# AlexandreRouma/SDRPlusPlus

Hardware: NVIDIA H100
Metric: complex IQ MSamples/s through FFT + 8-VFO WFM chain (higher is better)
Workload: dtype f32

## Files before the change

### sdrplusplus_b200/csrc/api.cpp

```cpp
#include "../../include/b200dsp.h"
#include "engine.h"
#include <chrono>
#include <map>
#include <cmath>
#include <cstdio>
#include <cstring>
#include <cstdlib>
#include <algorithm>

using namespace b200;

static int g_device = -1;

static int ensure_device() {
    int n = 0;
    cudaError_t e = cudaGetDeviceCount(&n);
    if (e != cudaSuccess || n <= 0) {
        set_error("no usable CUDA device (%s): libb200dsp has no CPU fallback", e == cudaSuccess ? "0 devices" : cudaGetErrorString(e));
        cudaGetLastError();
        return B200_ENODEV;
    }
    if (g_device < 0) { g_device = 0; }
    B200_CK(cudaSetDevice(g_device));
    return 0;
// ... 417 lines not shown
extern "C" int b200_fe_vfo_max_out(b200_fe* fe, int id, int count) {
    VfoSlot* v = get_vfo(fe, id);
    if (!v) { return B200_EINVAL; }
    return v->chain.max_out(count);
}
extern "C" int b200_fe_fft_max_lines(b200_fe* fe, int count) {
    if (!fe || !fe->fft_on) { return 0; }
    return (int)(count / ((long long)fe->fft.nz + fe->skip)) + 2;
}
extern "C" long long b200_fe_launch_count(b200_fe* fe) { return fe ? fe->sch.launches : 0; }
extern int g_xd_tma_launches;
extern "C" long long b200_fe_stat(b200_fe* fe, const char* key) {
    if (!fe || !key) { return -1; }
    if (!strcmp(key, "launches")) { return fe->sch.launches; }
    if (!strcmp(key, "s1_tma_launches")) { return g_xd_tma_launches; }
    if (!strcmp(key, "chunks")) { return (long long)fe->nsub; }
    if (!strcmp(key, "host_ns_plan")) { return fe->host_ns[0]; }
    if (!strcmp(key, "host_ns_fft")) { return fe->host_ns[1]; }
    if (!strcmp(key, "host_ns_run")) { return fe->host_ns[2]; }
    if (!strcmp(key, "host_ns_join")) { return fe->host_ns[3]; }
    if (!strcmp(key, "graph_hits")) { return fe->sch.graph_hits; }
    if (!strcmp(key, "graph_misses")) { return fe->sch.graph_misses; }
    if (!strcmp(key, "graphs")) { return (long long)fe->sch.graphs.size(); }
    if (!strcmp(key, "host_ns_stage1")) { return fe->sch.host_ns[0]; }
    if (!strcmp(key, "host_ns_tail")) { return fe->sch.host_ns[1]; }
    return -1;
}
extern "C" int b200_fe_set_option(b200_fe* fe, const char* key, int value) {
    if (!fe || !key) { set_error("null argument"); return B200_EINVAL; }
    if (!strcmp(key, "s1")) { fe->sch.s1_variant = value; return 0; }
    if (!strcmp(key, "overlap")) {
        if (b200_fe_vfo_count(fe) > 0) { set_error("'overlap' must be chosen before VFOs are added"); return B200_ESTATE; }
        if (cudaDeviceSynchronize() != cudaSuccess) { return cuda_fail(cudaGetLastError(), "sync"); }
        fe->sch.tail_stream = value ? fe->tail_stream : nullptr;
        return 0;
    }
    if (!strcmp(key, "pair")) { fe->sch.pair_conjugates = value != 0; return 0; }
    if (!strcmp(key, "fft_async")) { fe->fft_async = value != 0; return 0; }
    if (!strcmp(key, "s1_mt")) { kernels_set_xd_tile(value); return 0; }
    if (!strcmp(key, "s1_cps")) { kernels_set_xd_cps(value); return 0; }
    if (!strcmp(key, "s1_stages")) { kernels_set_xd_tma_stages(value); return 0; }
    if (!strcmp(key, "s1_diag")) { kernels_set_xd_tma_diag(value); return 0; }
    if (!strcmp(key, "s1_ctas")) { kernels_set_xd_tma_ctas(value); return 0; }
    if (!strcmp(key, "tails") || !strncmp(key, "ft_", 3)) {
        if (b200_fe_vfo_count(fe) > 0) { set_error("'%s' must be chosen before VFOs are added", key); return B200_ESTATE; }
        if (!strcmp(key, "tails")) { kernels_set_tail_variant(value >= 1 ? 1 : 0); fe->sch.fuse.on = value >= 2; return 0; }
        if (!strcmp(key, "ft_ob")) { fe->sch.fuse.ob_force = value; return 0; }
        if (!strcmp(key, "ft_obmax")) { fe->sch.fuse.ob_max = value; return 0; }
        if (!strcmp(key, "ft_smem_kb")) { fe->sch.fuse.smem_limit = value * 1024; return 0; }
        if (!strcmp(key, "ft_threads")) { fe->sch.fuse.threads = value; return 0; }
        if (!strcmp(key, "ft_direct")) { fe->sch.fuse.direct = value != 0; return 0; }
        if (!strcmp(key, "ft_prereg")) { fe->sch.fuse.pre_reg = value; return 0; }
        if (!strcmp(key, "ft_regall")) { fe->sch.fuse.reg_all = value != 0; return 0; }
// ... 1127 lines not shown
```

### sdrplusplus_b200/csrc/engine.cpp

```cpp
#include "engine.h"
#include <chrono>
#include "../../include/b200dsp.h"
#include <cmath>
#include <cstdarg>
#include <cstdio>
#include <cstring>
#include <algorithm>
#include <map>
#include <functional>
#include <cstdlib>

namespace b200 {

static thread_local char g_err[512] = "";
void set_error(const char* fmt, ...) {
    va_list ap;
    va_start(ap, fmt);
    vsnprintf(g_err, sizeof(g_err), fmt, ap);
    va_end(ap);
}
const char* last_error() { return g_err; }
int cuda_fail(cudaError_t e, const char* what) {
    set_error("CUDA error %d (%s) in %s", (int)e, cudaGetErrorString(e), what);
    if (e == cudaErrorNoDevice || e == cudaErrorInsufficientDriver) { return B200_ENODEV; }
// ... 288 lines not shown
    memset(init_state, 0, sizeof(init_state));
    init_state[7] = 1.0f;
    int rc = state.alloc(sizeof(init_state));
    if (rc) { return rc; }
    B200_CK(cudaMemcpy(state.p, init_state, sizeof(init_state), cudaMemcpyHostToDevice));
    return 0;
}
int FmIfStage::configure(int nbins) {
    if (!fmif_supported(nbins)) { set_error("FM IF noise reduction: %d bins (supported: 2 ... %d)", nbins, 64); return B200_EINVAL; }
    bins = nbins;
    hist = bins - 1;
    const std::vector<float> w = fmif_window(bins), t = dft_twiddles(bins);
    int rc;
    if ((rc = win.alloc(w.size() * sizeof(float), false)) || (rc = tw.alloc(t.size() * sizeof(float), false))) { return rc; }
    B200_CK(cudaMemcpy(win.p, w.data(), w.size() * sizeof(float), cudaMemcpyHostToDevice));
    B200_CK(cudaMemcpy(tw.p, t.data(), t.size() * sizeof(float), cudaMemcpyHostToDevice));
    return 0;
}

int Chain::finalize(int max_in, bool dbl_first, const FuseCfg* fuse) {
    if (st.empty()) { set_error("empty chain"); return B200_EINVAL; }
    int cap = max_in;
    if (dbl_first && st.size() >= 2 && st[0]->kind == K_XD) { st[1]->dbl = true; }
    for (auto& s : st) {
        if (s->kind != K_XD) {
            int rc = s->alloc_in(cap);
            if (rc) { return rc; }
        }
        else { s->cap_in = cap; }
        cap = s->max_out(cap);
    }
    {
        int c2 = max_in;
        for (auto& s : st) {
            if (s->kind == K_STEREO) {
                StereoStage* q = (StereoStage*)s.get();
                int rc2;
                if ((rc2 = q->p.alloc(((size_t)c2 + 8) * sizeof(float2), false)) || (rc2 = q->vco.alloc(((size_t)c2 + 8) * sizeof(float2), false))) { return rc2; }
            }
            c2 = s->max_out(c2);
        }
    }
    out_es = st.back()->out_es;
    out_cap = cap;
    int rc = out.alloc(((size_t)cap + 8) * out_es * sizeof(float));
    if (rc) { return rc; }
// ... 663 lines not shown
    }
    for (Chain* c : chains) {
        for (auto& sp : c->st) { sp->par = parity; }
    }
    if (tail_stream && chunk_idx >= 2) {
        B200_CK(cudaStreamWaitEvent(stream, ev_tail[parity], 0));
    }
    trace_mark("stage1 start", stream);
    for (Chain* c : chains) {
        depth = std::max(depth, c->st.size());
        for (size_t i = 0; i < c->st.size(); i++) {
            Stage* s = c->st[i].get();
            s->out_ptr = (i + 1 < c->st.size()) ? c->st[i + 1]->in_data() : (c->out_override ? c->out_override : c->out.as<float>());
            if (s->kind == K_XD) {
                XdStage* x = (XdStage*)s;
                if (x->taps_dirty) {
                    int rc = x->upload_taps(stream);
                    if (rc) { return rc; }
                }
            }
        }
    }
    std::map<int, std::vector<XdStage*>> groups;
    for (Chain* c : chains) {
        if (c->raw_input()) {
            XdStage* x = (XdStage*)c->st[0].get();
            groups[x->D].push_back(x);
        }
    }
    for (auto& kv : groups) {
        std::vector<XdStage*>& g = kv.second;
        for (size_t b = 0; b < g.size(); b += B200_BATCH) {
            XdParams p;
            memset(&p, 0, sizeof(p));
            p.in = raw;
            p.hist = raw_hist.as<float2>();
            p.hist_len = RAW_HIST;
            p.count = count;
            p.D = kv.first;
            p.in_scale = in_scale;
            p.QP = 1;
            p.njobs = (int)std::min<size_t>(B200_BATCH, g.size() - b);
            for (int v = 0; v < p.njobs; v++) {
                XdStage* x = g[b + v];
                p.job[v].out = (float2*)x->out_ptr;
                p.job[v].gpad = x->gpad.as<float2>();
                p.job[v].phase0 = x->chunk_phase0;
                p.job[v].w = x->w;
                p.job[v].offset = x->chunk_offset;
                p.job[v].n_out = x->n_out;
                p.job[v].T = x->T;
                p.job[v].h = x->hdev.as<float>();
                p.job[v].w_prev = x->chunk_w_prev;
                p.job[v].retuned = x->chunk_retuned ? 1 : 0;
// ... 42 lines not shown
                            const unsigned long long r = g[b + v]->w * (unsigned long long)P;
                            const double d0 = (double)(long long)r;
                            const double d1 = (double)(long long)(r - 0x8000000000000000ULL);
                            int sv = 0;
                            if (std::fabs(d0) <= tol) { sv = 1; } else if (std::fabs(d1) <= tol) { sv = -1; }
                            if (sv == 0 || (sg != 0 && sv != sg)) { ok = false; }
                            sg = sv;
                        }
                        if (!ok) { continue; }
                        for (int PS : { 8, 10 }) {
                            if (PS % P == 0) {
                                p.pfb_ps = PS;
                                p.pfb_sigma = (sg < 0 && ((PS / P) & 1)) ? -1 : 1;
                                break;
                            }
                        }
                    }
                }
            }
            int variant = s1_variant;
            for (int v = 0; v < p.njobs; v++) {
                if (g[b + v]->gpad_len < (p.D - 1) + (p.QP + 8) * p.D) { variant = 0; }
            }
            int nl = 0;
            cudaEvent_t t1 = timer_begin(0, stream);
            cudaError_t e = launch_xlate_decim(p, fmt, variant, stream, &nl);
            if (e != cudaSuccess) { return cuda_fail(e, "launch_xlate_decim"); }
            if (t1) { B200_CK(cudaEventRecord(t1, stream)); }
            trace_mark("stage1 done", stream);
            e = launch_xd_edge(p, fmt, stream, &nl);
            if (e != cudaSuccess) { return cuda_fail(e, "launch_xd_edge"); }
            launches += nl;
        }
    }
    if (carry_raw && count > 0) {
        CarryParams rc1;
        rc1.njobs = 1;
        CarryJob& j = rc1.job[0];
        j.dst = raw_hist.as<float>(); j.a = raw_hist.as<float>(); j.b = raw;
        j.h = RAW_HIST; j.la = RAW_HIST; j.lb = count; j.esize = 2; j.bfmt = fmt; j.scale = in_scale;
        cudaError_t e = launch_carry(rc1, stream);
        if (e != cudaSuccess) { return cuda_fail(e, "launch_carry"); }
        launches++;
    }
    if (tail_stream) {
        B200_CK(cudaEventRecord(ev_stage1[parity], stream));
        B200_CK(cudaStreamWaitEvent(ts, ev_stage1[parity], 0));
    }
    trace_mark("tails start", ts);
// ... 26 lines not shown
            int rc = dfr_flush();
            if (rc) { return rc; }
        }
        if (dfr.njobs == 0) {
            dfr_D = f->decim; dfr_T = f->ntaps; dfr_taps = &f->htaps;
            memcpy(dfr.taps, f->htaps.data(), (size_t)f->ntaps * sizeof(float));
        }
        FirJob& j = dfr.job[dfr.njobs++];
        j.in = (const float2*)f->base(); j.out = (float2*)f->out_ptr; j.taps = f->taps.as<float>();
        j.ntaps = f->ntaps; j.decim = f->decim; j.offset = f->chunk_offset; j.n_out = f->n_out;
        dfr.max_out = std::max(dfr.max_out, f->n_out);
        return 0;
    };
    auto dfr_ok = [&](const Stage* s) {
        if (fuse.pre_reg <= 0 || s->kind != K_FIRC || s->in_es != 2) { return false; }
        const FirCStage* f = (const FirCStage*)s;
        return f->decim > 1 && f->ntaps <= DFR_MAXT && dfir_reg_supported(f->decim, f->ntaps);
    };
    {
        int max_beg = 1;
        for (Chain* c : chains) { if (c->fp.active) { max_beg = std::max(max_beg, c->fp.beg); } }
        for (int lvl = 1; lvl < max_beg; lvl++) {
            for (Chain* c : chains) {
                if (!c->fp.active || lvl >= c->fp.beg) { continue; }
                FirCStage* f = (FirCStage*)c->st[lvl].get();
                if (f->n_out <= 0) { continue; }
                int rc = dfr_push(f);
                if (rc) { return rc; }
            }
            int rc = dfr_flush();
            if (rc) { return rc; }
        }
    }
    {
        std::vector<Chain*> fc;
        for (Chain* c : chains) {
            if (c->fp.active && c->st[c->fp.beg]->n_in > 0) { fc.push_back(c); }
        }
        if (!fc.empty()) {
            const int threads = (fuse.threads == 512 || fuse.threads == 256) ? fuse.threads : 128;
            size_t smem = 0;
            int ob_cap = 1 << 30;
            for (Chain* c : fc) { smem = std::max(smem, c->fp.smem); ob_cap = std::min(ob_cap, c->fp.ob_max); }
            static std::map<std::pair<int, size_t>, int> occ_cache;
            int cps;
            {
                auto key = std::make_pair(threads, smem);
// ... 110 lines not shown
            else {
                cudaError_t e = launch_squelch(sqp, ts, &nl);
                if (e != cudaSuccess) { return cuda_fail(e, "launch_squelch"); }
            }
            launches += nl;
            sqp.njobs = 0; sqp.max_n = 0;
            return 0;
        };
        auto st_flush = [&]() -> int {
            if (stp.njobs == 0) { return 0; }
            int nl = 0;
            if (g_rec) { g_rec->add(LaunchRec::T_STEREO, nullptr, &stp, sizeof(stp)); }
            else {
                cudaError_t e = launch_stereo(stp, ts, &nl);
                if (e != cudaSuccess) { return cuda_fail(e, "launch_stereo"); }
            }
            launches += nl;
            stp.njobs = 0; stp.max_n = 0;
            return 0;
        };
        for (Chain* c : chains) {
            if (lvl >= c->st.size()) { continue; }
            if (c->fp.active && lvl >= 1 && (int)lvl < c->fp.end) { continue; }
            Stage* s = c->st[lvl].get();
            int rc = 0;
            switch (s->kind) {
            case K_XD: break;
            case K_FIRC: {
                FirCStage* f = (FirCStage*)s;
                if (f->n_out <= 0) { break; }
                if (dfr_ok(f)) { rc = dfr_push(f); break; }
                if (fuse.pre_reg > 0 && f->decim == 1 && f->in_es == 2 && f->ntaps <= 2000 && f->chunk_offset == 0) {
                    FirJob& jr = fpr.job[fpr.njobs++];
                    jr.in = (const float2*)f->base(); jr.out = (float2*)f->out_ptr; jr.taps = f->taps.as<float>();
                    jr.ntaps = f->ntaps; jr.decim = 1; jr.offset = 0; jr.n_out = f->n_out;
                    fpr.max_out = std::max(fpr.max_out, f->n_out);
                    if (fpr.njobs == B200_BATCH) { rc = flush_batch(fpr, launch_fir_reg, ts, launches); fpr.max_out = 0; }
                    break;
                }
                FirJob& j = fp.job[fp.njobs++];
                j.in = (const float2*)f->base(); j.out = (float2*)f->out_ptr; j.taps = f->taps.as<float>();
                j.ntaps = f->ntaps; j.decim = f->decim; j.offset = f->chunk_offset; j.n_out = f->n_out;
                fp.max_out = std::max(fp.max_out, f->n_out);
                if (fp.njobs == B200_BATCH) { rc = flush_batch(fp, launch_fir_c, ts, launches); fp.max_out = 0; }
                break;
            }
// ... 126 lines not shown
        if ((rc = flush_batch(fp, launch_fir_c, ts, launches))) { return rc; }
        if ((rc = flush_batch(pp, launch_poly, ts, launches))) { return rc; }
        if ((rc = flush_batch(qp, launch_quad, ts, launches))) { return rc; }
        if ((rc = flush_batch(rp, launch_fir_r, ts, launches))) { return rc; }
        if ((rc = flush_batch(sp, launch_seq, ts, launches))) { return rc; }
        if ((rc = flush_batch(mp, launch_m2s, ts, launches))) { return rc; }
        if ((rc = flush_batch(cp2, launch_scale, ts, launches))) { return rc; }
        if ((rc = flush_batch(fmp, launch_fmif, ts, launches))) { return rc; }
        if ((rc = flush_batch(xlp, launch_rxl, ts, launches))) { return rc; }
        if ((rc = st_flush())) { return rc; }
        if ((rc = sq_flush())) { return rc; }
    }
    CarryParams cp;
    zero_params(cp, use_rec);
    auto push = [&](const CarryJob& j) -> int {
        cp.job[cp.njobs++] = j;
        if (cp.njobs == CARRY_BATCH) { return flush_batch(cp, launch_carry, ts, launches); }
        return 0;
    };
    for (Chain* c : chains) {
        for (auto& sp : c->st) {
            Stage* s = sp.get();
            if (s->kind == K_XD || s->hist <= 0 || s->fmid) { continue; }
            if (s->n_in <= 0 && !s->dbl) { continue; }
            CarryJob j;
            memset(&j, 0, sizeof(j));
            j.dst = s->other_base(); j.a = s->base(); j.b = s->in_data();
            j.h = s->hist; j.la = s->hist; j.lb = s->n_in; j.esize = s->in_es; j.bfmt = -1; j.scale = 0.0f;
            int rc = push(j);
            if (rc) { return rc; }
        }
    }
    int rcf = flush_batch(cp, launch_carry, ts, launches);
    if (rcf) { return rcf; }
    return 0;
    };
    if (nsplit == 1) {
        rec.cur_branch = 0;
        int rcs = tail_section(all_chains);
        if (rcs) { return rcs; }
    }
    else {
        const size_t half = (all_chains.size() + 1) / 2;
        std::vector<Chain*> ga(all_chains.begin(), all_chains.begin() + half), gb(all_chains.begin() + half, all_chains.end());
        rec.cur_branch = 0;
        int rcs = tail_section(ga);
// ... 20 lines not shown
```

### sdrplusplus_b200/csrc/engine.h

```cpp
#pragma once
#include <cuda_runtime.h>
#include <cstdint>
#include <memory>
#include <mutex>
#include <string>
#include <vector>
#include <unordered_map>
#include "kernels.cuh"
#include "design.h"

namespace b200 {

void trace_mark(const char* label, cudaStream_t s);
void trace_dump(const char* title);
bool trace_on();

void set_error(const char* fmt, ...);
const char* last_error();
int cuda_fail(cudaError_t e, const char* what);
#define B200_CK(call)                                                     \
    do {                                                                  \
        cudaError_t _e = (call);                                          \
        if (_e != cudaSuccess) { return b200::cuda_fail(_e, #call); }     \
    } while (0)
// ... 164 lines not shown
    DevBuf win, tw;
    FmIfStage() { kind = K_FMIF; in_es = 2; out_es = 2; }
    int configure(int nbins);
    int plan(int n) override { n_in = n; n_out = n; return n; }
    int max_out(int n) const override { return n; }
};

struct ScaleStage : Stage {
    float gain = 1.0f;
    ScaleStage(int es, float g) { kind = K_SCALE; in_es = es; out_es = es; gain = g; }
    int plan(int n) override { n_in = n; n_out = n; return n; }
    int max_out(int n) const override { return n; }
};

struct Chain {
    std::vector<std::unique_ptr<Stage>> st;
    DevBuf out;
    int out_es = 2;
    int out_cap = 0;
    int n_out = 0;
    float* out_override = nullptr;
    bool raw_input() const { return !st.empty() && st[0]->kind == K_XD; }
    int chan_fir = -1;
    FusedPlan fp;
    FuseCfg fcfg;
    int plan_fused();
    int finalize(int max_in, bool dbl_first = false, const FuseCfg* fuse = nullptr);
    int plan(int n);
    int max_out(int n) const;
    int peek(int n) const;
    void reset_state();
    int add_rxvfo(double inSR, double outSR, double bw, double offset);
    int add_xlator(double offsetHz, double samplerate);
    int add_power_decim(int ratio);
    int add_resampler(double inSR, double outSR);
    int add_fir_c(const std::vector<float>& taps, int decim);
    int add_fir_r(const std::vector<float>& taps, bool stereo);
    int add_quad(double deviationHz, double samplerate);
    int add_wfm(double deviationHz, double samplerate, bool lowPass, bool stereo = false);
    int add_nfm(double samplerate, double bandwidth, bool lowPass);
    int add_am(int agcMode, double bandwidth, double attack, double decay, double dcRate, double samplerate);
    int add_ssb(int mode, double bandwidth, double samplerate, double attack, double decay);
    int add_deemph(double tau, double samplerate);
    int add_af_chain(double afSamplerate, double audioSamplerate, bool highPass, double deemphTau);
    int add_wfm_rds(double deviationHz, double samplerate);
    int add_noise_blanker(double rate, double level);
// ... 16 lines not shown
    int replay(cudaStream_t s, long long* nlaunch) const;
};

struct Scheduler {
    cudaStream_t stream = nullptr;
    cudaStream_t tail_stream = nullptr;
    cudaEvent_t ev_stage1[2] = { nullptr, nullptr }, ev_tail[2] = { nullptr, nullptr };
    unsigned long long chunk_idx = 0;
    cudaStream_t out_stream() const { return tail_stream ? tail_stream : stream; }
    int enable_overlap(cudaStream_t tail);
    long long launches = 0;
    int graph_tails = -1;
    int graph_max_count = 1 << 30;
    int tail_split = 1;
    cudaStream_t tail_stream2 = nullptr;
    struct GraphEntry { cudaGraphExec_t exec = nullptr; long long launches = 0; std::vector<unsigned char> key; };
    std::unordered_map<unsigned long long, GraphEntry> graphs;
    LaunchRec rec;
    long long graph_hits = 0, graph_misses = 0;
    void drop_graphs();
    int launch_recorded(cudaStream_t ts, bool may_graph);
    long long host_ns[4] = { 0, 0, 0, 0 };
    int s1_variant = 8;
    FuseCfg fuse;
    int sm_count = 132;
    float in_scale = 1.0f / 32768.0f;
    bool pair_conjugates = true;
    bool time_s1 = false;
    static const size_t TIMER_MAX = 512;
    struct Timer { std::vector<cudaEvent_t> ev; size_t used = 0; };
    Timer timers[3];
    cudaEvent_t timer_begin(int group, cudaStream_t s);
    int group_stats(int group, double* ms_total, int* launches);
    int s1_stats(double* ms_total, int* launches) { return group_stats(0, ms_total, launches); }
    ~Scheduler();
    DevBuf raw_hist;
    static const int RAW_HIST = 1024;
    static const int STAGE_SPARE = 72;
    int init_raw();
    int run(std::vector<Chain*>& chains, const void* raw, int fmt, int count, bool carry_raw);
    int apply_deferred(std::vector<Chain*>& chains);
    int reset_raw();
};

}
```

### sdrplusplus_b200/csrc/kernels.cu

```cuda
#include "kernels.cuh"
#include <unordered_map>
#include <mutex>
#include <math.h>
#include <string.h>
#include <algorithm>

template <int FMT>
__device__ __forceinline__ float2 load_iq(const void* __restrict__ p, long long i, float sc) {
    if (FMT == FMT_CF32) {
        return __ldg(reinterpret_cast<const float2*>(p) + i);
    }
    else if (FMT == FMT_CS16) {
        short2 v = __ldg(reinterpret_cast<const short2*>(p) + i);
        return make_float2((float)v.x * sc, (float)v.y * sc);
    }
    else {
        char2 v = __ldg(reinterpret_cast<const char2*>(p) + i);
        return make_float2((float)v.x * sc, (float)v.y * sc);
    }
}

template <int FMT>
__device__ __forceinline__ float2 load_x(const XdParams& p, long long i) {
    if (i >= 0) {
// ... 758 lines not shown

typedef CUresult (*PFN_tmap_encode)(CUtensorMap*, CUtensorMapDataType, cuuint32_t, void*, const cuuint64_t*, const cuuint64_t*,
                                    const cuuint32_t*, const cuuint32_t*, CUtensorMapInterleave, CUtensorMapSwizzle,
                                    CUtensorMapL2promotion, CUtensorMapFloatOOBfill);
static PFN_tmap_encode tmap_encode_fn() {
    static PFN_tmap_encode fn = nullptr;
    static bool tried = false;
    if (!tried) {
        tried = true;
        void* f = nullptr;
        cudaDriverEntryPointQueryResult q;
        if (cudaGetDriverEntryPoint("cuTensorMapEncodeTiled", &f, cudaEnableDefault, &q) == cudaSuccess && q == cudaDriverEntryPointSuccess) {
            fn = (PFN_tmap_encode)f;
        }
        else { cudaGetLastError(); }
    }
    return fn;
}
int g_xd_tma_launches = 0;
int g_xd_tma_stages = 2;
void kernels_set_xd_tma_stages(int n) { g_xd_tma_stages = (n == 3) ? 3 : 2; }
static int g_xd_tma_diag = 0;
void kernels_set_xd_tma_diag(int v) { g_xd_tma_diag = v & 3; }
template <int LOGD, int QC, int PS, int MT, int NST>
static cudaError_t launch_xd_tma_n(const XdParams& p, const XtGeom& g, const CUtensorMap& tm, cudaStream_t s) {
    using Lay = XtLay<LOGD, QC, MT>;
    const size_t smem = (size_t)NST * Lay::STAGE + ((size_t)B200_BATCH * (PS + 16) + (size_t)Lay::NW * B200_BATCH * 4) * sizeof(float2) +
                        2 * NST * sizeof(unsigned long long) + 1024;
    if ((int)smem > kernels_max_smem_optin()) { return cudaErrorInvalidValue; }
    static bool attr_set = false;
    if (!attr_set) {
        cudaError_t e = set_smem(k_xd_tma<LOGD, QC, PS, MT, NST>, smem);
        if (e != cudaSuccess) { return e; }
        attr_set = true;
    }
    int grid = num_sms();
    if (g_xd_tma_ctas > 0 && g_xd_tma_ctas < grid) { grid = g_xd_tma_ctas; }
    if (grid > g.ntiles) { grid = g.ntiles; }
    k_xd_tma<LOGD, QC, PS, MT, NST><<<grid, (Lay::NW + 1) * 32, smem, s>>>(p, g, tm);
    g_xd_tma_launches++;
    return cudaGetLastError();
}
template <int LOGD, int QC, int PS, int MT>
static cudaError_t launch_xd_tma_t(const XdParams& p, const XtGeom& g, const CUtensorMap& tm, cudaStream_t s) {
    return g_xd_tma_stages == 3 ? launch_xd_tma_n<LOGD, QC, PS, MT, 3>(p, g, tm, s) : launch_xd_tma_n<LOGD, QC, PS, MT, 2>(p, g, tm, s);
}
static bool try_xd_tma(const XdParams& p, cudaStream_t s, cudaError_t* err) {
    const int D = p.D, PS = p.pfb_ps;
    if ((PS != 8 && PS != 10) || (D != 32 && D != 64) || !p.taps_host) { return false; }
    if (((uintptr_t)p.in & 15) != 0) { return false; }
    PFN_tmap_encode enc = tmap_encode_fn();
    if (!enc) { return false; }
    const int T = p.job[0].T;
    const int a0 = p.job[0].offset - (T - 1);
    const int org = ((a0 % D) + D) % D;
    for (int v = 0; v < p.njobs; v++) {
        const int a = p.job[v].offset - (p.job[v].T - 1);
        if (p.job[v].T != T || a != a0 || p.job[v].n_out != p.job[0].n_out || p.job[v].n_out <= 0) { return false; }
    }
    const int QC = (T + (org & 1) + D - 1) / D;
    int sh = org & 1;
    for (int al = 16; al >= 2; al >>= 1) {
        const int c = org & (al - 1);
        if ((T + c + D - 1) / D == QC) { sh = c; break; }
    }
    if (QC * D > XT_MAXTAPS) { return false; }
    XtGeom g;
// ... 414 lines not shown
```

### sdrplusplus_b200/csrc/kernels.cuh

```cuda
#pragma once
#include <cuda_runtime.h>
#include <stdint.h>

#define B200_BATCH 16

enum { FMT_CF32 = 0, FMT_CS16 = 1, FMT_CS8 = 2 };

struct XdJob {
    float2* out;
    const float2* gpad;
    unsigned long long phase0;
    unsigned long long w;
    int offset;
    int n_out;
    int T;
    const float* h;
    unsigned long long w_prev;
    int retuned;
};
struct XdParams {
    const void* in;
    const float2* hist;
    int hist_len;
    int count;
    int D;
    int QP;
    int njobs;
    int nslots;
    signed char slot_a[B200_BATCH], slot_b[B200_BATCH];
    int pfb_ps, pfb_sigma;
    float in_scale;
    const float* taps_host;
    XdJob job[B200_BATCH];
};

struct FirJob {
    const float2* in;
    float2* out;
    const float* taps;
    int ntaps, decim, offset, n_out;
};
struct FirParams { int njobs; int max_out; FirJob job[B200_BATCH]; };

#define DFR_THREADS 128
#define DFR_MAXT 72

struct DfrParams {
    int njobs;
    int max_out;
    float taps[DFR_MAXT];
    FirJob job[B200_BATCH];
};

bool dfir_reg_supported(int D, int T);
cudaError_t launch_dfir_reg(const DfrParams& p, int D, int T, cudaStream_t s);

// ... 277 lines not shown
```

### sdrplusplus_b200/csrc/xd_tma.cuh

```cuda
#pragma once
#include <cuda.h>

#define XT_STAGES NST
#define XT_MAXTAPS 512

struct XtGeom {
    float g[XT_MAXTAPS];
    long long jmin;
    int ntiles;
    int org;
    int s;
    int cj;
    int rows_tma;
    int diag;
};

__device__ __forceinline__ void xt_mbar_init(unsigned bar, int count) {
    asm volatile("mbarrier.init.shared::cta.b64 [%0], %1;\n" ::"r"(bar), "r"(count) : "memory");
}
__device__ __forceinline__ void xt_mbar_wait(unsigned bar, unsigned parity) {
    asm volatile("{\n.reg .pred p;\nXT_WAIT_%=:\nmbarrier.try_wait.parity.shared::cta.b64 p, [%0], %1;\n@!p bra XT_WAIT_%=;\n}\n" ::"r"(bar), "r"(parity) : "memory");
}
__device__ __forceinline__ void xt_mbar_arrive(unsigned bar) {
    asm volatile("mbarrier.arrive.shared::cta.b64 _, [%0];\n" ::"r"(bar) : "memory");
// ... 30 lines not shown
    for (int rp = RP0; rp < RP1; rp++) {
#pragma unroll
        for (int q = 0; q <= QC; q++) {
            const unsigned addr = sb + (unsigned)((q & 1) * REGION) + (aoff[q >> 1] ^ (unsigned)((rp & 7) << 4));
            float4 x;
            asm volatile("ld.shared.v4.f32 {%0, %1, %2, %3}, [%4];\n" : "=f"(x.x), "=f"(x.y), "=f"(x.z), "=f"(x.w) : "r"(addr));
#pragma unroll
            for (int e = 0; e < 2; e++) {
                const int r = 2 * rp + e;
                const float2 xe = e ? make_float2(x.z, x.w) : make_float2(x.x, x.y);
                if (q < QC) {
                    const float t = g.g[q * D + r];
                    S[0][(q * D + r) % PS] = ffma2(make_float2(t, t), xe, S[0][(q * D + r) % PS]);
                }
                if (q >= 1) {
                    const float t = g.g[(q - 1) * D + r];
                    S[1][((q - 1) * D + r) % PS] = ffma2(make_float2(t, t), xe, S[1][((q - 1) * D + r) % PS]);
                }
            }
        }
    }
}

template <int LOGD, int QC, int PS, int MT, int NST>
__global__ void __launch_bounds__((MT / 64 + 1) * 32, 1)
k_xd_tma(const __grid_constant__ XdParams p, const __grid_constant__ XtGeom g, const __grid_constant__ CUtensorMap tm) {
    using Lay = XtLay<LOGD, QC, MT>;
    constexpr int D = Lay::D, NSEG = Lay::NSEG, NR = Lay::NR, REGION = Lay::REGION, STAGE = Lay::STAGE, NW = Lay::NW;
    constexpr int NQH = (QC >> 1) + 1;
    constexpr int NSLOT = NST;
    constexpr int SLOT = STAGE;
    extern __shared__ __align__(1024) unsigned char xt_smem[];
    const unsigned sbase = ((unsigned)__cvta_generic_to_shared(xt_smem) + 1023u) & ~1023u;
    unsigned char* const gbase = xt_smem + (sbase - (unsigned)__cvta_generic_to_shared(xt_smem));
    float2* C = reinterpret_cast<float2*>(gbase + XT_STAGES * STAGE);
    float2* TL = C + (size_t)B200_BATCH * PS;
    float2* PHW = TL + (size_t)B200_BATCH * 16;
    unsigned long long* bars = reinterpret_cast<unsigned long long*>(PHW + (size_t)NW * B200_BATCH * 4);
    const unsigned bar0 = (unsigned)__cvta_generic_to_shared(bars);

    const int tid = threadIdx.x, lane = tid & 31, warp = tid >> 5;

    if (tid == 0) {
        for (int s = 0; s < NSLOT; s++) {
            xt_mbar_init(bar0 + 8 * s, 1);
            xt_mbar_init(bar0 + 8 * (NSLOT + s), NW);
        }
        asm volatile("fence.mbarrier_init.release.cluster;\n" ::: "memory");
    }
    __syncthreads();
    if (warp < NW) {
        for (int idx = tid; idx < p.njobs * PS; idx += NW * 32) {
            const int v = idx / PS, b = idx - v * PS;
            int a = (b - g.s) % PS;
            if (a < 0) { a += PS; }
            C[idx] = phasor_u64(p.job[v].w * (unsigned long long)a);
        }
        for (int idx = tid; idx < p.njobs * 16; idx += NW * 32) {
            const int v = idx >> 4, j = idx & 15;
            TL[idx] = phasor_u64(p.job[v].w * (unsigned long long)((long long)j * D));
        }
        asm volatile("bar.sync 1, %0;\n" ::"n"(NW * 32) : "memory");
    }

    auto tile_fast = [&](long long J0) { return J0 >= 0 && (J0 >> 1) + Lay::NEED <= (long long)g.rows_tma; };

    if (warp == NW) {
        if (lane == 0 && !(g.diag & 2)) {
            const unsigned long long pol = xt_policy_evict_first();
            int it = 0;
            for (int tile = blockIdx.x; tile < g.ntiles; tile += gridDim.x) {
                const long long J0 = g.jmin + (long long)tile * MT;
                const int row0 = (int)(J0 >> 1);
                const int sl = it % NSLOT;
                const unsigned ph = (unsigned)((it / NSLOT) & 1);
                it++;
                xt_mbar_wait(bar0 + 8 * (NSLOT + sl), ph ^ 1u);
                const unsigned full = bar0 + 8 * sl;
                xt_mbar_expect(full, (unsigned)SLOT);
                const unsigned dst = sbase + (unsigned)(sl * SLOT);
#pragma unroll
                for (int sg = 0; sg < NSEG; sg++) {
#pragma unroll
                    for (int par = 0; par < 2; par++) {
                        xt_tma_2d(dst + (unsigned)((sg * 2 + par) * REGION), &tm, full, par * 2 * D + sg * 32, row0, pol);
                    }
                }
            }
        }
        return;
    }

    const int jl = warp * 64 + 2 * lane;
    unsigned aoff[NQH];
#pragma unroll
    for (int qh = 0; qh < NQH; qh++) {
        const unsigned row = (unsigned)((jl >> 1) + qh);
        aoff[qh] = row * 128u + ((row & 7u) << 4);
    }
    int it = 0;
    for (int tile = blockIdx.x; tile < g.ntiles; tile += gridDim.x) {
        const long long J0 = g.jmin + (long long)tile * MT;
        {
            for (int e = lane; e < p.njobs * 4; e += 32) {
                const int vv = e >> 2, i = e & 3;
                const XdJob& Jv = p.job[vv];
                const int a0 = Jv.offset - (Jv.T - 1);
                const long long im0 = (long long)a0 + (J0 + warp * 64 + i * 16 - (long long)g.cj) * D;
                unsigned long long dr = Jv.w * (unsigned long long)PS;
                if (p.pfb_sigma < 0) { dr -= 0x8000000000000000ULL; }
                const long long corr = (long long)dr * (long long)(Jv.T / (2 * PS));
                PHW[(warp * B200_BATCH + vv) * 4 + i] = phasor_u64(Jv.phase0 + Jv.w * (unsigned long long)im0 + (unsigned long long)corr);
            }
        }
        const bool fast = tile_fast(J0);

        float2 S[2][PS];
#pragma unroll
        for (int o = 0; o < 2; o++)
#pragma unroll
            for (int a = 0; a < PS; a++) { S[o][a] = make_float2(0.f, 0.f); }
        const int sl = it % NSLOT;
        const unsigned ph = (unsigned)((it / NSLOT) & 1);
        it++;
        if (!(g.diag & 2)) { xt_mbar_wait(bar0 + 8 * sl, ph); }
        const unsigned sb = sbase + (unsigned)(sl * SLOT);
        if (!fast && !g.diag) {
            const long long ibase = J0 * D + g.org;
            unsigned char* stg = gbase + sl * SLOT;
            constexpr int NSAMP = (MT + QC + 1) * D;
            const long long tensor_end = (long long)g.org + (long long)g.rows_tma * (2 * D);
            const long long front = (long long)g.org - ibase;
            const int head = (int)(front > 0 ? (front < NSAMP ? front : NSAMP) : 0);
            long long t0 = tensor_end - ibase, t1 = (long long)p.count - ibase;
            if (t0 < head) { t0 = head; }
            if (t1 > NSAMP) { t1 = NSAMP; }
            auto patch = [&](int idx) {
                const float2 v = load_x<FMT_CF32>(p, ibase + idx);
                const int j = idx >> LOGD, r = idx & (D - 1), row = j >> 1;
                const int off = ((r >> 4) * 2 + (j & 1)) * REGION + row * 128 + ((((r >> 1) & 7) ^ (row & 7)) << 4) + (r & 1) * 8;
                *reinterpret_cast<float2*>(stg + off) = v;
            };
            for (int idx = tid; idx < head; idx += NW * 32) { patch(idx); }
            for (long long idx = t0 + tid; idx < t1; idx += NW * 32) { patch((int)idx); }
            asm volatile("bar.sync 1, %0;\n" ::"n"(NW * 32) : "memory");
        }
        if (!(g.diag & 1)) {
            xt_accumulate<LOGD, QC, PS, REGION, 0, 8, NQH>(S, g, sb, aoff);
            xt_accumulate<LOGD, QC, PS, REGION, 8, 16, NQH>(S, g, sb + 2 * REGION, aoff);
            if constexpr (NSEG == 4) {
                xt_accumulate<LOGD, QC, PS, REGION, 16, 24, NQH>(S, g, sb + 4 * REGION, aoff);
                xt_accumulate<LOGD, QC, PS, REGION, 24, 32, NQH>(S, g, sb + 6 * REGION, aoff);
            }
        }
        static_assert(NSEG == 2 || NSEG == 4, "D = 32 or 64");
        __syncwarp();
        if (lane == 0 && !(g.diag & 2)) { xt_mbar_arrive(bar0 + 8 * (NSLOT + sl)); }

        if (g.diag & 1) { continue; }
        const long long m0 = J0 + jl - (long long)g.cj;
        const int nout = p.job[0].n_out;
        const bool ok0 = m0 >= 0 && m0 < nout, ok1 = (m0 + 1) >= 0 && (m0 + 1) < nout;
        const int ih = (2 * lane) >> 4, il = (2 * lane) & 15;
        for (int sl = 0; sl < p.nslots; sl++) {
            const int ja = p.slot_a[sl], jb = p.slot_b[sl];
            float2 A0 = make_float2(0.f, 0.f), B0 = A0, A1 = A0, B1 = A0;
            const float2* cv = C + ja * PS;
#pragma unroll
            for (int a = 0; a < PS; a++) {
                const float2 c = cv[a];
                A0 = ffma2(make_float2(c.x, c.x), S[0][a], A0);
                B0 = ffma2(make_float2(c.y, c.y), S[0][a], B0);
                A1 = ffma2(make_float2(c.x, c.x), S[1][a], A1);
                B1 = ffma2(make_float2(c.y, c.y), S[1][a], B1);
            }
            {
                const float2 pc = PHW[(warp * B200_BATCH + ja) * 4 + ih];
                const float2 p0 = cmulf(pc, TL[ja * 16 + il]), p1 = cmulf(pc, TL[ja * 16 + il + 1]);
                float2* out = p.job[ja].out + m0;
                if (ok0) { out[0] = cmulf(make_float2(A0.x - B0.y, A0.y + B0.x), p0); }
                if (ok1) { out[1] = cmulf(make_float2(A1.x - B1.y, A1.y + B1.x), p1); }
            }
            if (jb >= 0) {
                const float2 pc = PHW[(warp * B200_BATCH + jb) * 4 + ih];
                const float2 p0 = cmulf(pc, TL[jb * 16 + il]), p1 = cmulf(pc, TL[jb * 16 + il + 1]);
                float2* out = p.job[jb].out + m0;
                if (ok0) { out[0] = cmulf(make_float2(A0.x + B0.y, A0.y - B0.x), p0); }
                if (ok1) { out[1] = cmulf(make_float2(A1.x + B1.y, A1.y - B1.x), p1); }
            }
        }
        __syncwarp();
    }
}
```

Measured before the change: 94600.

## Fold second-stage decimating FIR into the TMA xlate-decimate kernel

Adds a fused path where the stage-1 TMA translate/decimate kernel also runs the following decimate-by-4, 27-tap complex FIR. The intermediate output is staged in shared memory instead of being written to global memory and re-read by a separate FIR launch. Each CTA handles a contiguous run of tiles, with a warm-up tile to rebuild FIR history, and carries the history across chunks itself. The standalone FIR and its carry job are skipped for folded chains. The cost is extra shared memory, redundant warm-up compute per CTA, possible waits on the previous tail stream, and lower grid-stride parallelism.

```diff
diff --git a/sdrplusplus_b200/csrc/api.cpp b/sdrplusplus_b200/csrc/api.cpp
--- a/sdrplusplus_b200/csrc/api.cpp
+++ b/sdrplusplus_b200/csrc/api.cpp
@@ -463,6 +463,7 @@
     if (!strcmp(key, "graph_hits")) { return fe->sch.graph_hits; }
     if (!strcmp(key, "graph_misses")) { return fe->sch.graph_misses; }
     if (!strcmp(key, "graphs")) { return (long long)fe->sch.graphs.size(); }
+    if (!strcmp(key, "s1_folds")) { return fe->sch.s1_folds; }
     if (!strcmp(key, "host_ns_stage1")) { return fe->sch.host_ns[0]; }
     if (!strcmp(key, "host_ns_tail")) { return fe->sch.host_ns[1]; }
     return -1;
@@ -470,6 +471,7 @@
 extern "C" int b200_fe_set_option(b200_fe* fe, const char* key, int value) {
     if (!fe || !key) { set_error("null argument"); return B200_EINVAL; }
     if (!strcmp(key, "s1")) { fe->sch.s1_variant = value; return 0; }
+    if (!strcmp(key, "s1_fold")) { fe->sch.s1_fold = value != 0; return 0; }
     if (!strcmp(key, "overlap")) {
         if (b200_fe_vfo_count(fe) > 0) { set_error("'overlap' must be chosen before VFOs are added"); return B200_ESTATE; }
         if (cudaDeviceSynchronize() != cudaSuccess) { return cuda_fail(cudaGetLastError(), "sync"); }
diff --git a/sdrplusplus_b200/csrc/engine.cpp b/sdrplusplus_b200/csrc/engine.cpp
--- a/sdrplusplus_b200/csrc/engine.cpp
+++ b/sdrplusplus_b200/csrc/engine.cpp
@@ -334,6 +334,11 @@
     if (st.empty()) { set_error("empty chain"); return B200_EINVAL; }
     int cap = max_in;
     if (dbl_first && st.size() >= 2 && st[0]->kind == K_XD) { st[1]->dbl = true; }
+    if (st.size() >= 3 && st[0]->kind == K_XD && st[1]->kind == K_FIRC && st[1]->in_es == 2 && st[2]->in_es == 2 &&
+        xd_fold_supported(((FirCStage*)st[1].get())->decim, ((FirCStage*)st[1].get())->ntaps)) {
+        st[1]->dbl = true;
+        st[2]->dbl = true;
+    }
     for (auto& s : st) {
         if (s->kind != K_XD) {
             int rc = s->alloc_in(cap);
@@ -1043,14 +1048,20 @@
         }
     }
     std::map<int, std::vector<XdStage*>> groups;
+    std::map<int, std::vector<Chain*>> group_chains;
     for (Chain* c : chains) {
+        c->s1_folded_prev = c->s1_folded;
+        c->s1_folded = false;
         if (c->raw_input()) {
             XdStage* x = (XdStage*)c->st[0].get();
             groups[x->D].push_back(x);
-        }
-    }
+            group_chains[x->D].push_back(c);
+        }
+    }
+    bool waited_prev_tail = false;
     for (auto& kv : groups) {
         std::vector<XdStage*>& g = kv.second;
+        std::vector<Chain*>& gc = group_chains[kv.first];
         for (size_t b = 0; b < g.size(); b += B200_BATCH) {
             XdParams p;
             memset(&p, 0, sizeof(p));
@@ -1139,9 +1150,42 @@
             for (int v = 0; v < p.njobs; v++) {
                 if (g[b + v]->gpad_len < (p.D - 1) + (p.QP + 8) * p.D) { variant = 0; }
             }
+            XtFoldReq fold;
+            bool want_fold = s1_fold && variant >= 8 && fmt == FMT_CF32 && p.pfb_ps > 0;
+            for (int v = 0; v < p.njobs && want_fold; v++) {
+                Chain* c = gc[b + v];
+                if (c->st.size() < 3 || c->st[1]->kind != K_FIRC || !c->st[1]->dbl || !c->st[2]->dbl || g[b + v]->chunk_retuned ||
+                    (c->fp.active && c->fp.beg < 2)) { want_fold = false; break; }
+                FirCStage* f = (FirCStage*)c->st[1].get();
+                const FirCStage* f0 = (const FirCStage*)gc[b]->st[1].get();
+                if (!xd_fold_supported(f->decim, f->ntaps) || f->ntaps > XT_FOLD_MAXT || f->htaps != f0->htaps ||
+                    f->chunk_offset != f0->chunk_offset || f->n_out != f0->n_out) { want_fold = false; break; }
+                fold.f.off2 = f->chunk_offset;
+                fold.f.n_out2 = f->n_out;
+                fold.f.hist_rd[v] = (const float2*)f->base();
+                fold.f.hist_wr[v] = (float2*)f->other_base();
+                fold.f.out[v] = (float2*)f->out_ptr;
+            }
+            if (want_fold) {
+                const FirCStage* f0 = (const FirCStage*)gc[b]->st[1].get();
+                fold.D2 = f0->decim;
+                fold.T2 = f0->ntaps;
+                memcpy(fold.f.taps, f0->htaps.data(), (size_t)f0->ntaps * sizeof(float));
+                p.fold = &fold;
+                bool wait = false;
+                for (int v = 0; v < p.njobs; v++) { wait = wait || !gc[b + v]->s1_folded_prev; }
+                if (wait && tail_stream && chunk_idx >= 1 && !waited_prev_tail) {
+                    B200_CK(cudaStreamWaitEvent(stream, ev_tail[parity ^ 1], 0));
+                    waited_prev_tail = true;
+                }
+            }
             int nl = 0;
             cudaEvent_t t1 = timer_begin(0, stream);
             cudaError_t e = launch_xlate_decim(p, fmt, variant, stream, &nl);
+            if (fold.done) {
+                for (int v = 0; v < p.njobs; v++) { gc[b + v]->s1_folded = true; }
+                s1_folds++;
+            }
             if (e != cudaSuccess) { return cuda_fail(e, "launch_xlate_decim"); }
             if (t1) { B200_CK(cudaEventRecord(t1, stream)); }
             trace_mark("stage1 done", stream);
@@ -1214,7 +1258,7 @@
         for (Chain* c : chains) { if (c->fp.active) { max_beg = std::max(max_beg, c->fp.beg); } }
         for (int lvl = 1; lvl < max_beg; lvl++) {
             for (Chain* c : chains) {
-                if (!c->fp.active || lvl >= c->fp.beg) { continue; }
+                if (!c->fp.active || lvl >= c->fp.beg || (lvl == 1 && c->s1_folded)) { continue; }
                 FirCStage* f = (FirCStage*)c->st[lvl].get();
                 if (f->n_out <= 0) { continue; }
                 int rc = dfr_push(f);
@@ -1371,6 +1415,7 @@
         for (Chain* c : chains) {
             if (lvl >= c->st.size()) { continue; }
             if (c->fp.active && lvl >= 1 && (int)lvl < c->fp.end) { continue; }
+            if (lvl == 1 && c->s1_folded) { continue; }
             Stage* s = c->st[lvl].get();
             int rc = 0;
             switch (s->kind) {
@@ -1543,6 +1588,7 @@
         for (auto& sp : c->st) {
             Stage* s = sp.get();
             if (s->kind == K_XD || s->hist <= 0 || s->fmid) { continue; }
+            if (c->s1_folded && s == c->st[1].get()) { continue; }
             if (s->n_in <= 0 && !s->dbl) { continue; }
             CarryJob j;
             memset(&j, 0, sizeof(j));
diff --git a/sdrplusplus_b200/csrc/engine.h b/sdrplusplus_b200/csrc/engine.h
--- a/sdrplusplus_b200/csrc/engine.h
+++ b/sdrplusplus_b200/csrc/engine.h
@@ -210,6 +210,7 @@
     float* out_override = nullptr;
     bool raw_input() const { return !st.empty() && st[0]->kind == K_XD; }
     int chan_fir = -1;
+    bool s1_folded = false, s1_folded_prev = false;
     FusedPlan fp;
     FuseCfg fcfg;
     int plan_fused();
@@ -272,6 +273,8 @@
     int launch_recorded(cudaStream_t ts, bool may_graph);
     long long host_ns[4] = { 0, 0, 0, 0 };
     int s1_variant = 8;
+    int s1_fold = 1;
+    long long s1_folds = 0;
     FuseCfg fuse;
     int sm_count = 132;
     float in_scale = 1.0f / 32768.0f;
diff --git a/sdrplusplus_b200/csrc/kernels.cu b/sdrplusplus_b200/csrc/kernels.cu
--- a/sdrplusplus_b200/csrc/kernels.cu
+++ b/sdrplusplus_b200/csrc/kernels.cu
@@ -804,27 +804,40 @@
 void kernels_set_xd_tma_stages(int n) { g_xd_tma_stages = (n == 3) ? 3 : 2; }
 static int g_xd_tma_diag = 0;
 void kernels_set_xd_tma_diag(int v) { g_xd_tma_diag = v & 3; }
-template <int LOGD, int QC, int PS, int MT, int NST>
+template <int LOGD, int QC, int PS, int MT, int NST, int D2 = 0, int T2 = 0>
 static cudaError_t launch_xd_tma_n(const XdParams& p, const XtGeom& g, const CUtensorMap& tm, cudaStream_t s) {
     using Lay = XtLay<LOGD, QC, MT>;
-    const size_t smem = (size_t)NST * Lay::STAGE + ((size_t)B200_BATCH * (PS + 16) + (size_t)Lay::NW * B200_BATCH * 4) * sizeof(float2) +
-                        2 * NST * sizeof(unsigned long long) + 1024;
+    constexpr size_t NJ = D2 > 0 ? XT_FOLD_MAXJ : B200_BATCH;
+    const size_t smem = (size_t)NST * Lay::STAGE + (NJ * (PS + 16) + (size_t)Lay::NW * NJ * 4) * sizeof(float2) +
+                        2 * NST * sizeof(unsigned long long) + (D2 > 0 ? XtFoldLay<(D2 > 0 ? D2 : 1), (D2 > 0 ? T2 : 1), MT>::BYTES : 0) + 1024;
     if ((int)smem > kernels_max_smem_optin()) { return cudaErrorInvalidValue; }
     static bool attr_set = false;
     if (!attr_set) {
-        cudaError_t e = set_smem(k_xd_tma<LOGD, QC, PS, MT, NST>, smem);
+        cudaError_t e = set_smem(k_xd_tma<LOGD, QC, PS, MT, NST, D2, T2>, smem);
         if (e != cudaSuccess) { return e; }
         attr_set = true;
     }
     int grid = num_sms();
     if (g_xd_tma_ctas > 0 && g_xd_tma_ctas < grid) { grid = g_xd_tma_ctas; }
     if (grid > g.ntiles) { grid = g.ntiles; }
-    k_xd_tma<LOGD, QC, PS, MT, NST><<<grid, (Lay::NW + 1) * 32, smem, s>>>(p, g, tm);
+    typename XtFoldSel<D2>::type f;
+    memset(&f, 0, sizeof(f));
+    if constexpr (D2 > 0) {
+        f = p.fold->f;
+        f.run = cdiv(g.ntiles, grid);
+        grid = cdiv(g.ntiles, f.run);
+        p.fold->done = true;
+    }
+    k_xd_tma<LOGD, QC, PS, MT, NST, D2, T2><<<grid, (Lay::NW + 1) * 32, smem, s>>>(p, g, tm, f);
     g_xd_tma_launches++;
     return cudaGetLastError();
 }
+bool xd_fold_supported(int D2, int T2) { return D2 == 4 && T2 == 27; }
 template <int LOGD, int QC, int PS, int MT>
 static cudaError_t launch_xd_tma_t(const XdParams& p, const XtGeom& g, const CUtensorMap& tm, cudaStream_t s) {
+    if constexpr (LOGD == 5 && QC == 5 && MT == 256) {
+        if (p.fold && xd_fold_supported(p.fold->D2, p.fold->T2) && p.njobs <= XT_FOLD_MAXJ && g_xd_tma_stages != 3) { return launch_xd_tma_n<LOGD, QC, PS, MT, 2, 4, 27>(p, g, tm, s); }
+    }
     return g_xd_tma_stages == 3 ? launch_xd_tma_n<LOGD, QC, PS, MT, 3>(p, g, tm, s) : launch_xd_tma_n<LOGD, QC, PS, MT, 2>(p, g, tm, s);
 }
 static bool try_xd_tma(const XdParams& p, cudaStream_t s, cudaError_t* err) {
diff --git a/sdrplusplus_b200/csrc/kernels.cuh b/sdrplusplus_b200/csrc/kernels.cuh
--- a/sdrplusplus_b200/csrc/kernels.cuh
+++ b/sdrplusplus_b200/csrc/kernels.cuh
@@ -31,7 +31,24 @@
     int pfb_ps, pfb_sigma;
     float in_scale;
     const float* taps_host;
+    struct XtFoldReq* fold;
     XdJob job[B200_BATCH];
+};
+
+#define XT_FOLD_MAXT 28
+struct XtFold {
+    int run;
+    int off2, n_out2;
+    float taps[XT_FOLD_MAXT];
+    const float2* hist_rd[B200_BATCH];
+    float2* hist_wr[B200_BATCH];
+    float2* out[B200_BATCH];
+};
+bool xd_fold_supported(int D2, int T2);
+struct XtFoldReq {
+    int D2 = 0, T2 = 0;
+    bool done = false;
+    XtFold f = {};
 };
 
 struct FirJob {
diff --git a/sdrplusplus_b200/csrc/xd_tma.cuh b/sdrplusplus_b200/csrc/xd_tma.cuh
--- a/sdrplusplus_b200/csrc/xd_tma.cuh
+++ b/sdrplusplus_b200/csrc/xd_tma.cuh
@@ -76,24 +76,95 @@
     }
 }
 
-template <int LOGD, int QC, int PS, int MT, int NST>
+#define XT_FOLD_MAXJ 8
+template <int D2, int T2, int MT>
+struct XtFoldLay {
+    static constexpr int H = T2 - 1;
+    static constexpr int SP = ((MT + H + D2 - 1) / D2 + 1) & ~1;
+    static constexpr int STG = XT_FOLD_MAXJ * D2 * SP;
+    static constexpr size_t BYTES = (size_t)STG * sizeof(float2);
+};
+struct XtNoFold { int unused; };
+template <int D2> struct XtFoldSel { using type = XtFold; };
+template <> struct XtFoldSel<0> { using type = XtNoFold; };
+
+template <int D2, int T2, int MT>
+__device__ __forceinline__ void xt_fold_put(const XtFold& f, float2* STG, int n1, int v, float2 y0v, float2 y1v, long long y0, int jl,
+                                            bool first, bool warm) {
+    using FL = XtFoldLay<D2, T2, MT>;
+    constexpr int H = FL::H, SP = FL::SP;
+    float2* row = STG + v * D2 * SP;
+#pragma unroll
+    for (int e = 0; e < 2; e++) {
+        const long long m = y0 + jl + e;
+        float2 x = e ? y1v : y0v;
+        if (m < 0) { x = (m + H >= 0) ? f.hist_rd[v][m + H] : make_float2(0.f, 0.f); }
+        else if (m >= n1) { x = make_float2(0.f, 0.f); }
+        else if (!warm && m >= n1 - H) { f.hist_wr[v][m - (n1 - H)] = x; }
+        const int P = H + jl + e, at = (P % D2) * SP + P / D2;
+        if (P >= MT && !first) { row[at - MT / D2] = row[at]; }
+        row[at] = x;
+    }
+}
+template <int D2, int T2, int MT, int R0>
+__device__ __forceinline__ void xt_fold_fir(const XtFold& f, const float2* STG, int njobs, int b, int o, long long j) {
+    using FL = XtFoldLay<D2, T2, MT>;
+    constexpr int SP = FL::SP, NV = XT_FOLD_MAXJ / 2;
+    const float2* row[NV];
+#pragma unroll
+    for (int i = 0; i < NV; i++) {
+        const int v = b + 2 * i;
+        row[i] = STG + (v < njobs ? v : 0) * D2 * SP + o;
+    }
+    float2 acc[NV];
+#pragma unroll
+    for (int i = 0; i < NV; i++) { acc[i] = make_float2(0.0f, 0.0f); }
+#pragma unroll
+    for (int k = 0; k < T2; k++) {
+        const float h = f.taps[k];
+        const int at = ((R0 + k) % D2) * SP + (R0 + k) / D2;
+#pragma unroll
+        for (int i = 0; i < NV; i++) { acc[i] = ffma2(make_float2(h, h), row[i][at], acc[i]); }
+    }
+    if (j >= 0 && j < f.n_out2) {
+#pragma unroll
+        for (int i = 0; i < NV; i++) {
+            if (b + 2 * i < njobs) { f.out[b + 2 * i][j] = acc[i]; }
+        }
+    }
+}
+
+template <int LOGD, int QC, int PS, int MT, int NST, int D2, int T2>
 __global__ void __launch_bounds__((MT / 64 + 1) * 32, 1)
-k_xd_tma(const __grid_constant__ XdParams p, const __grid_constant__ XtGeom g, const __grid_constant__ CUtensorMap tm) {
+k_xd_tma(const __grid_constant__ XdParams p, const __grid_constant__ XtGeom g, const __grid_constant__ CUtensorMap tm,
+         const __grid_constant__ typename XtFoldSel<D2>::type f) {
     using Lay = XtLay<LOGD, QC, MT>;
     constexpr int D = Lay::D, NSEG = Lay::NSEG, NR = Lay::NR, REGION = Lay::REGION, STAGE = Lay::STAGE, NW = Lay::NW;
     constexpr int NQH = (QC >> 1) + 1;
     constexpr int NSLOT = NST;
     constexpr int SLOT = STAGE;
+    constexpr bool FOLD = D2 > 0;
+    using FL = XtFoldLay<(FOLD ? D2 : 1), (FOLD ? T2 : 1), MT>;
+    static_assert(!FOLD || (NW * 32 == 2 * (MT / D2) && T2 <= XT_FOLD_MAXT && MT % D2 == 0), "one thread per output position and VFO pair");
+    constexpr int NJ = FOLD ? XT_FOLD_MAXJ : B200_BATCH;
     extern __shared__ __align__(1024) unsigned char xt_smem[];
     const unsigned sbase = ((unsigned)__cvta_generic_to_shared(xt_smem) + 1023u) & ~1023u;
     unsigned char* const gbase = xt_smem + (sbase - (unsigned)__cvta_generic_to_shared(xt_smem));
     float2* C = reinterpret_cast<float2*>(gbase + XT_STAGES * STAGE);
-    float2* TL = C + (size_t)B200_BATCH * PS;
-    float2* PHW = TL + (size_t)B200_BATCH * 16;
-    unsigned long long* bars = reinterpret_cast<unsigned long long*>(PHW + (size_t)NW * B200_BATCH * 4);
+    float2* TL = C + (size_t)NJ * PS;
+    float2* PHW = TL + (size_t)NJ * 16;
+    unsigned long long* bars = reinterpret_cast<unsigned long long*>(PHW + (size_t)NW * NJ * 4);
     const unsigned bar0 = (unsigned)__cvta_generic_to_shared(bars);
+    float2* STG = reinterpret_cast<float2*>(bars + 2 * NSLOT);
 
     const int tid = threadIdx.x, lane = tid & 31, warp = tid >> 5;
+    int t_beg = blockIdx.x, t_end = g.ntiles, t_step = gridDim.x, t_out = 0;
+    if constexpr (FOLD) {
+        t_out = blockIdx.x * f.run;
+        t_end = min(t_out + f.run, g.ntiles);
+        t_beg = t_out > 0 ? t_out - 1 : 0;
+        t_step = 1;
+    }
 
     if (tid == 0) {
         for (int s = 0; s < NSLOT; s++) {
@@ -114,6 +185,18 @@
             const int v = idx >> 4, j = idx & 15;
             TL[idx] = phasor_u64(p.job[v].w * (unsigned long long)((long long)j * D));
         }
+        if constexpr (FOLD) {
+            if (t_beg == 0) {
+                const long long y0 = g.jmin - g.cj;
+                const int n1 = p.job[0].n_out;
+                for (int idx = tid; idx < p.njobs * FL::H; idx += NW * 32) {
+                    const int v = idx / FL::H, i = idx - v * FL::H;
+                    const long long h = y0 + i;
+                    STG[(v * D2 + i % D2) * FL::SP + i / D2] = h >= 0 ? f.hist_rd[v][h] : make_float2(0.f, 0.f);
+                    if (n1 + i < FL::H) { f.hist_wr[v][i] = f.hist_rd[v][n1 + i]; }
+                }
+            }
+        }
         asm volatile("bar.sync 1, %0;\n" ::"n"(NW * 32) : "memory");
     }
 
@@ -123,7 +206,7 @@
         if (lane == 0 && !(g.diag & 2)) {
             const unsigned long long pol = xt_policy_evict_first();
             int it = 0;
-            for (int tile = blockIdx.x; tile < g.ntiles; tile += gridDim.x) {
+            for (int tile = t_beg; tile < t_end; tile += t_step) {
                 const long long J0 = g.jmin + (long long)tile * MT;
                 const int row0 = (int)(J0 >> 1);
                 const int sl = it % NSLOT;
@@ -153,8 +236,9 @@
         aoff[qh] = row * 128u + ((row & 7u) << 4);
     }
     int it = 0;
-    for (int tile = blockIdx.x; tile < g.ntiles; tile += gridDim.x) {
+    for (int tile = t_beg; tile < t_end; tile += t_step) {
         const long long J0 = g.jmin + (long long)tile * MT;
+        const bool warm = FOLD && tile < t_out, work = !warm || warp == NW - 1;
         {
             for (int e = lane; e < p.njobs * 4; e += 32) {
                 const int vv = e >> 2, i = e & 3;
@@ -164,7 +248,7 @@
                 unsigned long long dr = Jv.w * (unsigned long long)PS;
                 if (p.pfb_sigma < 0) { dr -= 0x8000000000000000ULL; }
                 const long long corr = (long long)dr * (long long)(Jv.T / (2 * PS));
-                PHW[(warp * B200_BATCH + vv) * 4 + i] = phasor_u64(Jv.phase0 + Jv.w * (unsigned long long)im0 + (unsigned long long)corr);
+                PHW[(warp * NJ + vv) * 4 + i] = phasor_u64(Jv.phase0 + Jv.w * (unsigned long long)im0 + (unsigned long long)corr);
             }
         }
         const bool fast = tile_fast(J0);
@@ -199,7 +283,7 @@
             for (long long idx = t0 + tid; idx < t1; idx += NW * 32) { patch((int)idx); }
             asm volatile("bar.sync 1, %0;\n" ::"n"(NW * 32) : "memory");
         }
-        if (!(g.diag & 1)) {
+        if (!(g.diag & 1) && work) {
             xt_accumulate<LOGD, QC, PS, REGION, 0, 8, NQH>(S, g, sb, aoff);
             xt_accumulate<LOGD, QC, PS, REGION, 8, 16, NQH>(S, g, sb + 2 * REGION, aoff);
             if constexpr (NSEG == 4) {
@@ -218,29 +302,64 @@
         const int ih = (2 * lane) >> 4, il = (2 * lane) & 15;
         for (int sl = 0; sl < p.nslots; sl++) {
             const int ja = p.slot_a[sl], jb = p.slot_b[sl];
-            float2 A0 = make_float2(0.f, 0.f), B0 = A0, A1 = A0, B1 = A0;
-            const float2* cv = C + ja * PS;
-#pragma unroll
-            for (int a = 0; a < PS; a++) {
-                const float2 c = cv[a];
-                A0 = ffma2(make_float2(c.x, c.x), S[0][a], A0);
-                B0 = ffma2(make_float2(c.y, c.y), S[0][a], B0);
-                A1 = ffma2(make_float2(c.x, c.x), S[1][a], A1);
-                B1 = ffma2(make_float2(c.y, c.y), S[1][a], B1);
-            }
-            {
-                const float2 pc = PHW[(warp * B200_BATCH + ja) * 4 + ih];
-                const float2 p0 = cmulf(pc, TL[ja * 16 + il]), p1 = cmulf(pc, TL[ja * 16 + il + 1]);
-                float2* out = p.job[ja].out + m0;
-                if (ok0) { out[0] = cmulf(make_float2(A0.x - B0.y, A0.y + B0.x), p0); }
-                if (ok1) { out[1] = cmulf(make_float2(A1.x - B1.y, A1.y + B1.x), p1); }
-            }
-            if (jb >= 0) {
-                const float2 pc = PHW[(warp * B200_BATCH + jb) * 4 + ih];
-                const float2 p0 = cmulf(pc, TL[jb * 16 + il]), p1 = cmulf(pc, TL[jb * 16 + il + 1]);
-                float2* out = p.job[jb].out + m0;
-                if (ok0) { out[0] = cmulf(make_float2(A0.x + B0.y, A0.y - B0.x), p0); }
-                if (ok1) { out[1] = cmulf(make_float2(A1.x + B1.y, A1.y - B1.x), p1); }
+            float2 ya0 = make_float2(0.f, 0.f), ya1 = ya0, yb0 = ya0, yb1 = ya0;
+            if (work) {
+                float2 A0 = make_float2(0.f, 0.f), B0 = A0, A1 = A0, B1 = A0;
+                const float2* cv = C + ja * PS;
+#pragma unroll
+                for (int a = 0; a < PS; a++) {
+                    const float2 c = cv[a];
+                    A0 = ffma2(make_float2(c.x, c.x), S[0][a], A0);
+                    B0 = ffma2(make_float2(c.y, c.y), S[0][a], B0);
+                    A1 = ffma2(make_float2(c.x, c.x), S[1][a], A1);
+                    B1 = ffma2(make_float2(c.y, c.y), S[1][a], B1);
+                }
+                {
+                    const float2 pc = PHW[(warp * NJ + ja) * 4 + ih];
+                    const float2 p0 = cmulf(pc, TL[ja * 16 + il]), p1 = cmulf(pc, TL[ja * 16 + il + 1]);
+                    ya0 = cmulf(make_float2(A0.x - B0.y, A0.y + B0.x), p0);
+                    ya1 = cmulf(make_float2(A1.x - B1.y, A1.y + B1.x), p1);
+                    if constexpr (!FOLD) {
+                        float2* out = p.job[ja].out + m0;
+                        if (ok0) { out[0] = ya0; }
+                        if (ok1) { out[1] = ya1; }
+                    }
+                }
+                if (jb >= 0) {
+                    const float2 pc = PHW[(warp * NJ + jb) * 4 + ih];
+                    const float2 p0 = cmulf(pc, TL[jb * 16 + il]), p1 = cmulf(pc, TL[jb * 16 + il + 1]);
+                    yb0 = cmulf(make_float2(A0.x + B0.y, A0.y - B0.x), p0);
+                    yb1 = cmulf(make_float2(A1.x + B1.y, A1.y - B1.x), p1);
+                    if constexpr (!FOLD) {
+                        float2* out = p.job[jb].out + m0;
+                        if (ok0) { out[0] = yb0; }
+                        if (ok1) { out[1] = yb1; }
+                    }
+                }
+            }
+            if constexpr (FOLD) {
+                if (work) {
+                    xt_fold_put<D2, T2, MT>(f, STG, nout, ja, ya0, ya1, J0 - g.cj, jl, tile == t_beg, warm);
+                    if (jb >= 0) { xt_fold_put<D2, T2, MT>(f, STG, nout, jb, yb0, yb1, J0 - g.cj, jl, tile == t_beg, warm); }
+                }
+            }
+        }
+        if constexpr (FOLD) {
+            if (!warm) {
+                asm volatile("bar.sync 1, %0;\n" ::"n"(NW * 32) : "memory");
+                constexpr int NO = MT / D2;
+                const long long y0 = J0 - g.cj;
+                const int b = tid / NO, o = tid - b * NO;
+                const int r0 = (int)((((long long)f.off2 - y0) % D2 + D2) % D2);
+                const long long j = (y0 + r0 - f.off2) / D2 + o;
+                static_assert(D2 == 4, "staging offsets are instantiated for D2 = 4");
+                switch (r0) {
+                case 0: xt_fold_fir<D2, T2, MT, 0>(f, STG, p.njobs, b, o, j); break;
+                case 1: xt_fold_fir<D2, T2, MT, 1>(f, STG, p.njobs, b, o, j); break;
+                case 2: xt_fold_fir<D2, T2, MT, 2>(f, STG, p.njobs, b, o, j); break;
+                default: xt_fold_fir<D2, T2, MT, 3>(f, STG, p.njobs, b, o, j); break;
+                }
+                asm volatile("bar.sync 1, %0;\n" ::"n"(NW * 32) : "memory");
             }
         }
         __syncwarp();
```

Result: faster. 98420 (median of 6 runs) (+4.0%).
